# RozDavid/UnScene3D

Hardware: AMD Instinct MI355X
Metric: training scenes/sec (Res16UNet34C+Mask3D, 150k voxels) (higher is better)
Workload: dtype f32

## Files before the change

include/usc3d.h:

```cpp
#ifndef USC3D_H
#define USC3D_H

#include <stdint.h>

#ifdef __cplusplus
extern "C" {
#endif

typedef void* usc_stream_t;

enum usc_status {
  USC_OK = 0,
  USC_ERR_ARG = -1,
  USC_ERR_LAUNCH = -2,
  USC_ERR_RANGE = -3
};

const char* usc_last_error(void);
int usc_abi_version(void);
const char* usc_build_info(void);
int usc_device_count(void);


int usc_voxel_floor_f64(const double* xyz, int64_t n, double voxel_size,
// ... 288 lines not shown
                         void* ws, int64_t ws_bytes, usc_stream_t s);
int usc_bn_backward_reduce(const float* x, const float* dy, const float* y_out,
                           const float* mean, const float* invstd, int64_t n,
                           int32_t c, int32_t training, int32_t accumulate, float* dgamma,
                           float* dbeta, float* mean_g, float* mean_gxhat,
                           void* ws, int64_t ws_bytes, usc_stream_t s);
int usc_relu_fwd(const float* x, float* y, int64_t numel, usc_stream_t s);
int usc_relu_bwd(const float* y, const float* dy, float* dx, int64_t numel,
                 usc_stream_t s);

int usc_avgpool_down2(const float* in, int32_t c, const int32_t* nbr2,
                      int64_t n_coarse, float* out, usc_stream_t s);
int usc_avgpool_down2_ex(const float* in, int32_t c, int32_t ld,
                         const int64_t* row_of, const int32_t* nbr2,
                         int64_t n_coarse, float* out, uint8_t* mask_out,
                         usc_stream_t s);

int usc_gather_rows(const float* src, int32_t c, const int64_t* idx, int64_t n,
                    float* out, usc_stream_t s);

int usc_scatter_add_rows(const float* src, int32_t c, const int64_t* idx,
                         int64_t n, float* dst, usc_stream_t s);

int usc_scatter_rows_unique(const float* src, int32_t c, const int64_t* idx,
                            int64_t n, float* dst, usc_stream_t s);
int usc_scatter_rows_unique_add(const float* src, int32_t c, const int64_t* idx,
                                int64_t n, float* dst, usc_stream_t s);

int64_t usc_sample_keys_ws_bytes(int32_t n_scenes, int32_t K, int32_t q);
int usc_sample_keys(const float* feats, int32_t c, const uint8_t* mask, int32_t q, const float* pos, int32_t p,
                    const int64_t* idx, int32_t n_scenes, int32_t K, const int32_t* n_valid, float* out_feats,
                    uint8_t* out_mask, float* out_pos, void* ws, int64_t ws_bytes, usc_stream_t s);

int64_t usc_segment_csr_ws_bytes(int64_t n, int64_t S);
int usc_segment_csr(const int64_t* seg, int64_t n, int64_t S, int64_t* order,
                    int64_t* seg_off, void* ws, int64_t ws_bytes,
                    usc_stream_t s);
int usc_segment_mean_fwd(const float* src, int32_t c, const int64_t* order,
                         const int64_t* seg_off, int64_t S, float* out,
                         usc_stream_t s);
int usc_segment_mean_bwd(const float* dout, int32_t c, const int64_t* seg,
                         const int64_t* seg_off, int64_t n, float* dsrc,
                         usc_stream_t s);

int usc_segment_mean_nonzero(const float* feats, int32_t d,
                             const int64_t* order, const int64_t* seg_off,
                             int64_t S, float* out, int64_t* nonzero_cnt,
                             usc_stream_t s);
int usc_segment_max_nonzero(const float* feats, int32_t d,
                            const int64_t* order, const int64_t* seg_off,
                            int64_t S, float* out, int64_t* nonzero_cnt,
                            usc_stream_t s);

int32_t usc_attn_max_queries(void);
int32_t usc_attn_lse_stride(int32_t L);
int64_t usc_attn_ws_bytes(int32_t L, int32_t S, int32_t B, int32_t H);
int usc_attn_fwd(const float* q, const float* k, const float* v,
                 const uint8_t* mask, int32_t L, int32_t S, int32_t B, int32_t H,
                 int32_t E, float* o, float* lse, void* ws, int64_t ws_bytes,
                 usc_stream_t s);
int usc_attn_bwd(const float* q, const float* k, const float* v,
                 const uint8_t* mask, const float* o, const float* lse,
                 const float* dO, int32_t L, int32_t S, int32_t B, int32_t H,
                 int32_t E, float* dq, float* dk, float* dv,
                 int32_t mask_bits_in_ws ,
                 void* ws, int64_t ws_bytes, usc_stream_t s);
// ... 329 lines not shown
```

unscene3d_amd/_lib.py:

```python
from __future__ import annotations

import ctypes as C
import os

import torch

_HERE = os.path.dirname(os.path.abspath(__file__))
LIB_PATH = os.environ.get("USC3D_LIB") or os.path.join(_HERE, "libusc3d_hip.so")

_p = C.c_void_p
_i32 = C.c_int32
_i64 = C.c_int64
_f64 = C.c_double
_f32 = C.c_float

class KMap(C.Structure):
    _fields_ = [("nbr", _p), ("perm", _p), ("tile_mask", _p), ("pair_in", _p), ("pair_out", _p), ("koff", _p),
                ("n_in", _i64), ("n_out", _i64), ("pair_capacity", _i64), ("K", _i32), ("reserved", _i32)]


class BNDesc(C.Structure):
    _fields_ = [("gamma", _p), ("beta", _p), ("running_mean", _p), ("running_var", _p), ("num_batches_tracked", _p),
                ("eps", _f32), ("momentum", _f32), ("c", _i32), ("training", _i32)]

# ... 81 lines not shown
    "usc_launch_stats_begin": (C.c_int, [_p, _i64, _p]),
    "usc_launch_stats_end": (_i64, [_p, _i64]),
    "usc_wall_clock_khz": (_i64, []),
    "usc_conv_ws_bytes": (_i64, [_kp, _i32, _i32, _i32]),
    "usc_unit_ws_bytes": (_i64, [_kp, _i32, _i32, _i32]),
    "usc_conv_forward": (C.c_int, [_kp, _i32, _p, _i32, _p, _i32, _p, _p, _p, _i64, _p]),
    "usc_conv_backward": (C.c_int, [_kp, _i32, _p, _i32, _p, _i32, _p, _p, _i32, _p, _i32, _p, _i64, _p]),
    "usc_bn_eval_stats": (C.c_int, [_p, _p, _p, _p, _f32, _i32, _p, _p, _p, _p, _p]),
    "usc_conv_bn_act_forward": (C.c_int, [_kp, _i32, _p, _i32, _p, _i32, _bp, _p, _i32, _p, _p, _p, _p, _i64, _p]),
    "usc_unit_bf16_ws_bytes": (_i64, [_kp, _i32, _i32, _i32]),
    "usc_conv_bn_act_forward_bf16": (C.c_int, [_kp, _i32, _p, _i32, _p, _i32, _bp, _p, _i32, _p, _p, _p, _p, _i64, _p]),
    "usc_unit_split_ws_bytes": (_i64, [_kp, _i32, _i32, _i32, _i32]),
    "usc_conv_bn_act_forward_split": (C.c_int, [_kp, _i32, _p, _i32, _p, _i32, _i32, _bp, _p, _i32, _p, _p, _p, _p, _i64, _p]),
    "usc_conv_bn_act_backward_split": (C.c_int, [_kp, _i32, _p, _i32, _p, _i32, _i32, _bp, _p, _p, _p, _p, _p, _p, _p, _i32, _p,
                                                 _i32, _p, _p, _i32, _p, _i64, _p]),
    "usc_conv_bn_act_backward": (C.c_int, [_kp, _i32, _p, _i32, _p, _i32, _bp, _p, _p, _p, _p, _p, _p, _p, _i32, _p,
                                           _i32, _p, _p, _i32, _p, _i64, _p]),
    "usc_colstats_ws_bytes": (_i64, [_i64, _i32]),
    "usc_colstats": (C.c_int, [_p, _p, _i64, _i32, _p, _p, _p, _i64, _p]),
    "usc_bn_apply": (C.c_int, [_p, _p, _p, _p, _i32, _p, _i64, _i32, _p]),
    "usc_bn_backward_dx": (C.c_int, [_p, _p, _p, _p, _p, _p, _p, _p, _p, _p, _i64, _i32, _p]),
    "usc_bn_backward_reduce": (C.c_int, [_p, _p, _p, _p, _p, _i64, _i32, _i32, _i32, _p, _p, _p, _p, _p, _i64, _p]),
    "usc_bn_forward_stats": (C.c_int, [_p, _i64, _i32, _p, _p, _f32, _f32, _p, _p, _p, _p, _p, _p, _p, _p, _i64, _p]),
    "usc_relu_fwd": (C.c_int, [_p, _p, _i64, _p]),
    "usc_relu_bwd": (C.c_int, [_p, _p, _p, _i64, _p]),
    "usc_avgpool_down2": (C.c_int, [_p, _i32, _p, _i64, _p, _p]),
    "usc_avgpool_down2_ex": (C.c_int, [_p, _i32, _i32, _p, _p, _i64, _p, _p, _p]),
    "usc_gather_rows": (C.c_int, [_p, _i32, _p, _i64, _p, _p]),
    "usc_scatter_add_rows": (C.c_int, [_p, _i32, _p, _i64, _p, _p]),
    "usc_scatter_rows_unique": (C.c_int, [_p, _i32, _p, _i64, _p, _p]),
    "usc_scatter_rows_unique_add": (C.c_int, [_p, _i32, _p, _i64, _p, _p]),
    "usc_sample_keys_ws_bytes": (_i64, [_i32, _i32, _i32]),
    "usc_sample_keys": (C.c_int, [_p, _i32, _p, _i32, _p, _i32, _p, _i32, _i32, _p, _p, _p, _p, _p, _i64, _p]),
    "usc_segment_csr_ws_bytes": (_i64, [_i64, _i64]),
    "usc_segment_csr": (C.c_int, [_p, _i64, _i64, _p, _p, _p, _i64, _p]),
    "usc_segment_mean_fwd": (C.c_int, [_p, _i32, _p, _p, _i64, _p, _p]),
    "usc_segment_mean_bwd": (C.c_int, [_p, _i32, _p, _p, _i64, _p, _p]),
    "usc_segment_mean_nonzero": (C.c_int, [_p, _i32, _p, _p, _i64, _p, _p, _p]),
    "usc_segment_max_nonzero": (C.c_int, [_p, _i32, _p, _p, _i64, _p, _p, _p]),
    "usc_ncut_similarity": (C.c_int, [_p, _i64, _i32, _i32, _p, _p, _p]),
    "usc_ncut_similarity_masked": (C.c_int, [_p, _p, _i64, _i32, _i32, _p, _p, _p]),
    "usc_ncut_normalize_mat": (C.c_int, [_p, _i64, _p, _i64, _p]),
    "usc_ncut_binarize": (C.c_int, [_p, _p, _i64, _f32, _f64, _p, _p, _p, _p]),
    "usc_ncut_fiedler_ws_bytes": (_i64, [_i64]),
    "usc_ncut_fiedler": (C.c_int, [_p, _p, _i64, _f64, _p, _p, _p, _i64, _p]),
    "usc_ncut_fiedler_ex": (C.c_int, [_p, _p, _i64, _f64, _p, _p, _p, _i64, _p, _i32]),
    "usc_ncut_fiedler_plan": (_i32, [_i64, _i32, _i32]),
    "usc_knn1": (C.c_int, [_p, _i64, _p, _i64, _p, _p, _p]),
    "usc_knn1_grid_ws_bytes": (_i64, [_i64, _p]),
    "usc_knn1_grid": (C.c_int, [_p, _i64, _p, _i64, _p, _f64, _p, _p, _p, _p, _i64, _p]),
    "usc_knn_hybrid_grid_ws_bytes": (_i64, [_i64, _p]),
    "usc_knn_hybrid_grid": (C.c_int, [_p, _i64, _p, _i64, _f32, _i32, _p, _f64, _p, _p, _p, _p, _i64, _p]),
    "usc_normals_pca": (C.c_int, [_p, _i64, _p, _i64, _p, _p, _i32, _p, _p]),
    "usc_cc_eps_init": (C.c_int, [_p, _i64, _p]),
    "usc_cc_eps_step": (C.c_int, [_p, _i64, _f32, _p, _p, _p, _p]),
    "usc_cc_eps_finish": (C.c_int, [_p, _i64, _p, _p, _p]),
    "usc_dbscan_cell_keys": (C.c_int, [_p, _i64, _f32, _f64, _f64, _f64, _i32, _i32, _i32, _p, _p]),
    "usc_dbscan_neighbor_table": (C.c_int, [_p, _i64, _i32, _i32, _i32, _p, _p]),
    "usc_dbscan_ws_bytes": (_i64, [_i64, _i32, _i64, _i32]),
    "usc_dbscan_labels": (C.c_int, [_p, _p, _p, _p, _p, _p, _i64, _i32, _i64, _f32, _i32, _p, _i64, _p, _p, _p]),
    "usc_dbscan_expand": (C.c_int, [_p, _p, _p, _i64, _i32, _i64, _p, _p]),
    "usc_project_planes_fwd": (C.c_int, [_p, _p, _p, _i64, _i32, _i32, _i32, _i32] + [_p] * 10),
    "usc_project_planes_bwd": (C.c_int, [_p, _i64, _i32, _i32, _i32, _i32, _p, _p, _p, _p, _p]),
    "usc_brick_mask_build": (C.c_int, [_p, _i64, _p, _i32, _i32, _i32, _i32, _p, _p]),
    "usc_raycast_first_hit_map": (C.c_int, [_p, _p, _i64, _i64, _p, _p, _i32, _i32, _i32, _p, _p, _i32, _i32, _i32, _i32,
                                            _f32, _f32, _f32, _p, _p, _p]),
# ... 133 lines not shown
```

unscene3d_amd/csrc/rows.hip:

```cpp
#include <math.h>
#include <stdlib.h>

#include "common.h"
#include "scan.h"

namespace usc {

void launch_group_reduce(const float* partial, int G, int64_t numel4, int cout, const float* bias, int accumulate,
                         float* out, hipStream_t st);

enum StatMode { STAT_XY = 0, STAT_BN_BWD = 1 };

struct StatArgs {
  const float* x;
  const float* y;
  const float* y_out;
  const float* mean;
  const float* invstd;
  int64_t n;
  int c;
};

constexpr int kStatMaxBlocks = 1024;
constexpr int kStatUnroll = 4;
// ... 519 lines not shown
  const int CT = c / VEC;
  const int64_t total = n_coarse * CT;
  for (int64_t j = (int64_t)blockIdx.x * blockDim.x + threadIdx.x; j < total; j += (int64_t)gridDim.x * blockDim.x) {
    const int64_t p = j / CT;
    const int cg = (int)(j - p * CT);
    float acc[VEC];
#pragma unroll
    for (int v = 0; v < VEC; ++v) acc[v] = 0.f;
    int cnt = 0;
#pragma unroll
    for (int k = 0; k < 8; ++k) {
      const int ch = nbr2[(int64_t)k * n_coarse + p];
      if (ch >= 0) {
        ++cnt;
        const int64_t row = row_of ? row_of[ch] : (int64_t)ch;
        if (VEC == 4) {
          const float4 t = *reinterpret_cast<const float4*>(in + row * ld + cg * 4);
          acc[0] += t.x; acc[1] += t.y; acc[2] += t.z; acc[3] += t.w;
        } else {
          acc[0] += in[row * ld + cg];
        }
      }
    }
    const float inv = 1.f / (float)(cnt > 0 ? cnt : 1);
    if (mask_out) {
#pragma unroll
      for (int v = 0; v < VEC; ++v) mask_out[p * c + cg * VEC + v] = (1.f / (1.f + expf(-(acc[v] * inv)))) < 0.5f;
    } else if (VEC == 4) {
      *reinterpret_cast<float4*>(out + p * c + cg * 4) =
          make_float4(acc[0] * inv, acc[1] * inv, acc[2] * inv, acc[3] * inv);
    } else {
      out[p * c + cg] = acc[0] * inv;
    }
  }
}

template <int VEC>
__global__ __launch_bounds__(256) void gather_rows_kernel(const float* __restrict__ src, int c,
                                                         const int64_t* __restrict__ idx, int64_t n,
                                                         float* __restrict__ out) {
  const int CT = c / VEC;
  const int64_t total = n * CT;
  for (int64_t j = (int64_t)blockIdx.x * blockDim.x + threadIdx.x; j < total; j += (int64_t)gridDim.x * blockDim.x) {
    const int64_t r = j / CT;
    const int cg = (int)(j - r * CT);
    const int64_t sr = idx[r];
    if (VEC == 4)
      *reinterpret_cast<float4*>(out + r * c + cg * 4) = *reinterpret_cast<const float4*>(src + sr * c + cg * 4);
    else
      out[r * c + cg] = src[sr * c + cg];
  }
}

constexpr int kSegTile = 1024;

__global__ __launch_bounds__(256) void seg_hist_kernel(const int64_t* __restrict__ seg, int64_t n, int64_t S,
                                                      int32_t* __restrict__ hist ) {
  const int64_t t = blockIdx.x;
  const int64_t b = t * kSegTile;
  for (int j = threadIdx.x; j < kSegTile; j += 256) {
    const int64_t i = b + j;
    if (i < n) atomicAdd(&hist[t * S + seg[i]], 1);
  }
}
__global__ __launch_bounds__(256) void seg_tilescan_kernel(int32_t* __restrict__ hist, int64_t T, int64_t S,
                                                          int32_t* __restrict__ counts) {
// ... 733 lines not shown
  USC_REQUIRE(n_scenes >= 1 && n_scenes <= usc::kSampleMaxScenes && K >= 1 && c >= 0 && c % 4 == 0 && q >= 0 &&
                  c <= 512 && q <= usc::kSampleMaxQ && (pos == nullptr || (p >= 4 && p % 4 == 0 && p <= 512)) &&
                  (c > 0 || q > 0),
              "usc_sample_keys: unsupported sizes (scenes <= 16, queries <= 256, channel counts multiples of 4 up to 512)");
  USC_REQUIRE(idx && n_valid && (c == 0 || (feats && out_feats)) && (q == 0 || (mask && out_mask && ws)) &&
                  (pos == nullptr || out_pos),
              "usc_sample_keys: null pointer");
  if (c == 0) { feats = nullptr; out_feats = nullptr; }
  if (q == 0) { mask = nullptr; out_mask = nullptr; }
  usc::SampleArgs a{};
  a.feats = feats; a.mask = mask; a.pos = pos; a.idx = idx;
  a.out_feats = out_feats; a.out_mask = out_mask; a.out_pos = out_pos; a.part = (unsigned char*)ws;
  a.c = c; a.q = q; a.p = p; a.K = K;
  a.nblk = (int)ceil_div((int64_t)K, (int64_t)usc::kSampleRows);
  a.qs = (q + 3) / 4 * 4;
  USC_REQUIRE(q == 0 || ((uintptr_t)ws & 3) == 0, "usc_sample_keys: workspace must be 4-byte aligned");
  USC_REQUIRE(q == 0 || ws_bytes >= usc_sample_keys_ws_bytes(n_scenes, K, q), "usc_sample_keys: workspace too small");
  for (int b = 0; b < n_scenes; ++b) {
    USC_REQUIRE(n_valid[b] >= 1, "usc_sample_keys: a scene without rows");
    a.n_valid[b] = n_valid[b];
  }
  const dim3 grid((unsigned)a.nblk, (unsigned)n_scenes);
  if (q <= 128) {
    hipLaunchKernelGGL(usc::sample_keys_kernel<1>, grid, dim3(256), 0, as_stream(s), a);
    if (q > 0) hipLaunchKernelGGL(usc::sample_fix_kernel<1>, grid, dim3(256), 0, as_stream(s), a);
  } else {
    hipLaunchKernelGGL(usc::sample_keys_kernel<2>, grid, dim3(256), 0, as_stream(s), a);
    hipLaunchKernelGGL(usc::sample_fix_kernel<2>, grid, dim3(256), 0, as_stream(s), a);
  }
  USC_CHECK_LAUNCH("usc_sample_keys");
  return USC_OK;
}

int usc_scatter_rows_unique(const float* src, int32_t c, const int64_t* idx, int64_t n, float* dst, usc_stream_t s) {
  USC_REQUIRE(c >= 1 && n >= 0, "usc_scatter_rows_unique: bad sizes");
  if (n == 0) return USC_OK;
  USC_REQUIRE(src && idx && dst, "usc_scatter_rows_unique: null pointer");
  if (c % 4 == 0)
    hipLaunchKernelGGL((usc::scatter_rows_kernel<4>), dim3(stream_grid(n * (c / 4), 256)), dim3(256), 0, as_stream(s), src,
                       (int)c, idx, n, dst);
  else
    hipLaunchKernelGGL((usc::scatter_rows_kernel<1>), dim3(stream_grid(n * c, 256)), dim3(256), 0, as_stream(s), src, (int)c,
                       idx, n, dst);
  USC_CHECK_LAUNCH("usc_scatter_rows_unique");
  return USC_OK;
}

int usc_scatter_rows_unique_add(const float* src, int32_t c, const int64_t* idx, int64_t n, float* dst, usc_stream_t s) {
  USC_REQUIRE(c >= 1 && n >= 0, "usc_scatter_rows_unique_add: bad sizes");
  if (n == 0) return USC_OK;
  USC_REQUIRE(src && idx && dst, "usc_scatter_rows_unique_add: null pointer");
  if (c % 4 == 0)
    hipLaunchKernelGGL((usc::scatter_rows_rmw_kernel<4>), dim3(stream_grid(n * (c / 4), 256)), dim3(256), 0, as_stream(s),
                       src, (int)c, idx, n, dst);
  else
    hipLaunchKernelGGL((usc::scatter_rows_rmw_kernel<1>), dim3(stream_grid(n * c, 256)), dim3(256), 0, as_stream(s), src,
                       (int)c, idx, n, dst);
  USC_CHECK_LAUNCH("usc_scatter_rows_unique_add");
  return USC_OK;
}

int usc_scatter_add_rows(const float* src, int32_t c, const int64_t* idx, int64_t n, float* dst, usc_stream_t s) {
  USC_REQUIRE(c >= 1 && n >= 0, "usc_scatter_add_rows: bad sizes");
  if (n == 0) return USC_OK;
  USC_REQUIRE(src && idx && dst, "usc_scatter_add_rows: null pointer");
  if (c % 4 == 0)
// ... 132 lines not shown
```

unscene3d_amd/models/mask3d.py:

```python
import contextlib
import os

import torch
import torch.nn as nn
from torch.nn import functional as F

from .. import MinkowskiEngine as ME
from .. import ops
from ..MinkowskiEngine import MinkowskiOps as me
from ..MinkowskiEngine.MinkowskiPooling import MinkowskiAvgPooling
from ..pointnet2_utils import furthest_point_sample
from .modules.common import conv
from .modules.helpers_3detr import GenericMLP
from .position_embedding import PositionEmbeddingCoordsSine

SINGLE_POINT_ERROR = "only a single point gives nans in cross-attention"


class Mask3D(nn.Module):
    def __init__(self, config, hidden_dim, num_queries, num_heads, dim_feedforward, sample_sizes, shared_decoder,
                 num_classes, num_decoders, dropout, pre_norm, positional_encoding_type, non_parametric_queries,
                 train_on_segments, normalize_pos_enc, use_level_embed, scatter_type, hlevels, use_np_features,
                 voxel_size, max_sample_size, random_queries, gauss_scale, random_query_both, random_normal):
        super().__init__()
# ... 319 lines not shown
                    elif plan["gidx"] is not None:
                        bufs = step_fn.input_buffers
                feats_l = aux[hlevel].F
                fused = (plan["gidx"] is not None and feats_l.is_cuda
                         and feats_l.dtype == torch.float32 and n_scenes <= 16 and feats_l.shape[1] % 4 == 0
                         and self.num_queries <= fused_attn_max_queries())

                on_side = use_side and fused
                if on_side:
                    for t in (plan["gidx"], samples["pos_keys"][pidx], feats_l):
                        if t is not None and t.is_cuda:
                            t.record_stream(side)
                with (torch.cuda.stream(side) if on_side else contextlib.nullcontext()):
                    if fused:
                        batched_aux = ops.sample_keys(
                            feats_l.contiguous(), None, None, plan["gidx"], n_scenes, curr_sample_size, n_valid,
                            unique=plan["all_sampled"], valid_unique=True,
                            sink=sinks.setdefault((hlevel, bool(plan["all_sampled"])), ops.GradSink()))
                    else:
                        batched_aux = _stack([ops.gather_rows(decomposed_aux[k].contiguous(), rand_idx[k],
                                                              unique=sizes[k] > curr_sample_size) for k in range(n_scenes)])
                    k_keys, v_keys = self._key_prep(dec, i)(batched_aux, samples["pos_keys"][pidx],
                                                            outs=None if bufs is None else (bufs[2], bufs[3]))
                    if on_side:
                        kv_done = torch.cuda.Event()
                        kv_done.record(side)
                        if bufs is None:
                            k_keys.record_stream(main)
                            v_keys.record_stream(main)

                normed, queries = self._norm_queries(queries)
                output_class, outputs_mask, attn_mask = self.mask_module(
                    queries, mask_features, mask_segments, len(aux) - hlevel - 1, ret_attn_mask=True,
                    point2segment=p2s_arg, coords=coords, defer_class=True, normed=normed)
                decomposed_attn = attn_mask.decomposed_features
                if fused and attn_mask.F.dtype == torch.bool and attn_mask.F.shape[1] <= fused_attn_max_queries():
                    batched_attn = ops.sample_keys(None, attn_mask.F.contiguous(), None, plan["gidx"], n_scenes,
                                                   curr_sample_size, n_valid,
                                                   outs=None if bufs is None else (None, bufs[4], None))
                else:
                    batched_attn = _stack([decomposed_attn[k][rand_idx[k], :] for k in range(n_scenes)])
                    batched_attn.permute(0, 2, 1)[batched_attn.sum(1) == curr_sample_size] = False
                    if not plan["all_sampled"]:
                        batched_attn = torch.logical_or(batched_attn, _stack(mask_idx)[..., None])
                    if bufs is not None:
                        bufs[4].copy_(batched_attn)
                        batched_attn = bufs[4]

                rec = getattr(self, "attn_mask_record", None)
                if rec is not None:
                    rec.append(batched_attn.detach().clone())
                if on_side:
                    main.wait_event(kv_done)
                queries = step_fn(queries, query_pos, k_keys, v_keys, batched_attn.contiguous())

                predictions_class.append(output_class)
                predictions_mask.append(outputs_mask)

        output_class, outputs_mask = self.mask_module(queries, mask_features, mask_segments, 0, ret_attn_mask=False,
                                                      point2segment=p2s_arg, coords=coords, defer_class=True)
        predictions_class.append(output_class)
        predictions_mask.append(outputs_mask)
        if early is not None:
            predictions_mask = _early_stage_gate(self, early, pcd_features, mask_features, seg_csr, predictions_mask)
        predictions_class = list(self.class_embed_head(torch.stack(predictions_class)).unbind(0))

        return {
            "pred_logits": predictions_class[-1],
            "pred_masks": predictions_mask[-1],
            "aux_outputs": self._set_aux_loss(predictions_class, predictions_mask),
            "sampled_coords": _host_array(sampled_coords) if sampled_coords is not None else None,
            "backbone_features": pcd_features,
        }

    def _early_stage(self, pcd_features, aux, point2segment):
        from .. import program
        feats = pcd_features.F
        handle = program.handle_of(feats)
        if not (self.training and torch.is_grad_enabled() and self.train_on_segments and self.scatter_type == "mean"
                and not self.use_np_features and point2segment is not None and feats.is_cuda
                and feats.dtype == torch.float32 and self.mask_dim % 32 == 0 and (len(aux) - 1) not in self.hlevels
                and program.early_possible(handle)):
            return None
        head = self.mask_features_head
        bias = head.bias
        if head.kernel_volume != 1 or head.stride != 1 or ops._grad_target(head.kernel) is None:
            return None
        if bias is not None and not (bias.requires_grad and ops._grad_target(bias) is not None):
            return None
        cm = pcd_features.coordinate_manager
        if not all(isinstance(sl, slice) for sl in cm.batch_slices(pcd_features._ts())):
            return None
        return handle

    def _norm_queries(self, queries):
        norm = self.decoder_norm
        if (queries.is_cuda and queries.dtype == torch.float32 and queries.requires_grad
                and isinstance(norm, LayerNorm) and norm.elementwise_affine and norm.bias is not None
                and len(norm.normalized_shape) == 1 and norm.normalized_shape[0] in ops._LN_DIMS):
            return ops.layer_norm(queries, norm.weight, norm.bias, norm.eps, passthrough=True)
        return norm(queries), queries

    def mask_module(self, query_feat, mask_features, mask_segments, num_pooling_steps, ret_attn_mask=True,
                    point2segment=None, coords=None, defer_class=False, normed=None):
        query_feat = self.decoder_norm(query_feat) if normed is None else normed
        head = self.mask_embed_head
        Q = query_feat.shape[-2]
        q_pad = (-Q) % 32
        if query_feat.is_cuda and query_feat.dtype == torch.float32:
            if defer_class and query_feat.requires_grad:
                hidden, query_feat = ops.linear(query_feat, head[0].weight, head[0].bias, relu=True, passthrough=True)
            else:
                hidden = ops.linear(query_feat, head[0].weight, head[0].bias, relu=True)
            if (q_pad and query_feat.dim() == 3 and query_feat.shape[0] == 1
                    and isinstance(head[2], Linear) and head[2].out_features % 32 == 0):
                mask_embed = ops.linear(hidden, head[2].weight, head[2].bias, pad_rows_to=Q + q_pad)
                mask_embed = _PaddedRows(mask_embed, Q)
            else:
                mask_embed = head[2](hidden)
        else:
            mask_embed = head(query_feat)
        outputs_class = query_feat if defer_class else self.class_embed_head(query_feat)

        output_masks, output_segments = [], []
        if (point2segment is not None and ret_attn_mask and num_pooling_steps >= 1 and query_feat.is_cuda
                and _FUSED_ATTN_MASK):
            for i, seg_feat in enumerate(mask_segments):
                logits, mask_segments[i] = _mask_logits(seg_feat, mask_embed[i], chain=True)
                output_segments.append(logits)
            cm, ts = mask_features.coordinate_manager, mask_features._ts()
            if len(output_segments) == 1:
                pooled = output_segments[0].detach()
                rows = point2segment[0].to(torch.int64).contiguous()
            else:
                Q = output_segments[0].shape[1]
                pooled = torch.cat([getattr(o, "_usc_padded", o).detach() for o in output_segments])[:, :Q]
                rows = getattr(cm, "_usc_p2s_batched", None)
                if rows is None or rows.shape[0] != mask_features.F.shape[0]:
                    off, parts = 0, []
                    for p2s, seg in zip(point2segment, mask_segments):
                        parts.append(p2s.to(torch.int64) + off)
                        off += seg.shape[0]
                    rows = torch.cat(parts).contiguous()
                    cm._usc_p2s_batched = rows
            for step in range(num_pooling_steps):
                if step == 0:
                    pooled = ops.avgpool_down2(pooled, _child_segment_table(cm, ts, rows),
                                               threshold=num_pooling_steps == 1)
                else:
                    pooled = ops.avgpool_down2(pooled, cm.stride_map(ts)["nbr2"],
                                               threshold=step == num_pooling_steps - 1)
                ts *= 2
            attn_mask = me.SparseTensor(features=pooled, coordinate_manager=cm,
                                        coordinate_map_key=ME.CoordinateMapKey(ts))
            return outputs_class, output_segments, attn_mask
        if point2segment is not None:
            for i, seg_feat in enumerate(mask_segments):
                output_segments.append(_mask_logits(seg_feat, mask_embed[i]))
                if ret_attn_mask:
                    with torch.no_grad():
                        output_masks.append(ops.gather_rows(output_segments[-1].detach().contiguous(),
                                                            point2segment[i].to(torch.int64).contiguous()))
        else:
            per_scene = mask_features.decomposed_features
            for i in range(len(per_scene)):
                output_masks.append(_mask_logits(per_scene[i], mask_embed[i]))

        if ret_attn_mask:
            attn_mask = me.SparseTensor(features=torch.cat(output_masks).detach(),
                                        coordinate_manager=mask_features.coordinate_manager,
                                        coordinate_map_key=mask_features.coordinate_map_key)
            for _ in range(num_pooling_steps):
                attn_mask = self.pooling(attn_mask.float())
            attn_mask = me.SparseTensor(features=(attn_mask.F.detach().sigmoid() < 0.5),
                                        coordinate_manager=attn_mask.coordinate_manager,
                                        coordinate_map_key=attn_mask.coordinate_map_key)
            if point2segment is not None:
                return outputs_class, output_segments, attn_mask
            return outputs_class, output_masks, attn_mask
        if point2segment is not None:
            return outputs_class, output_segments
        return outputs_class, output_masks

    @torch.jit.unused
# ... 232 lines not shown
_KV_SIDE_STREAM = os.environ.get("USC3D_KV_SIDE_STREAM", "1") != "0"


def set_kv_side_stream(on: bool):
    global _KV_SIDE_STREAM
    if torch.cuda.is_available():
        torch.cuda.synchronize()
    _KV_SIDE_STREAM = bool(on)
_FUSED_ATTN_MASK = os.environ.get("USC3D_FUSED_ATTN_MASK", "1") != "0"
_FUSED_ATTN_WIDE = os.environ.get("USC3D_FUSED_ATTN_WIDE", "1") != "0"


def fused_attn_max_queries() -> int:
    return ops.ATTN_MAX_QUERIES if _FUSED_ATTN_WIDE else min(128, ops.ATTN_MAX_QUERIES)


_PAD_CACHE = {}


def _padded_index(n, size, device):
    key = (int(n), int(size), str(device))
    hit = _PAD_CACHE.get(key)
    if hit is None:
        if len(_PAD_CACHE) > 256:
            _PAD_CACHE.clear()
        idx = torch.zeros(size, dtype=torch.long, device=device)
        midx = torch.ones(size, dtype=torch.bool, device=device)
        idx[:n] = torch.arange(n, device=device)
        midx[:n] = False
        hit = _PAD_CACHE[key] = (idx, midx)
    return hit


def _child_segment_table(cm, ts, rows):
    cache = cm.__dict__.setdefault("_usc_child_segments", {})
    hit = cache.get(ts)
    if hit is None or hit[0] != rows.data_ptr():
        nbr2 = cm.stride_map(ts)["nbr2"]
        tab = torch.where(nbr2 >= 0, rows.to(torch.int32)[nbr2.clamp(min=0).long()], nbr2).contiguous()
        hit = cache[ts] = (rows.data_ptr(), tab, rows)
    return hit[1]


def _segment_max(feats, seg, S):
    out = torch.zeros((int(S), feats.shape[1]), dtype=feats.dtype, device=feats.device)
    return out.scatter_reduce(0, seg.to(torch.int64)[:, None].expand(-1, feats.shape[1]), feats, "amax", include_self=False)


def _stack(tensors):
    tensors = list(tensors)
    return tensors[0].unsqueeze(0) if len(tensors) == 1 else torch.stack(tensors)


def _col_minmax(x):
    mn, mx = torch.aminmax(x.t().contiguous(), dim=1)
    return mn, mx


def _residual_norm(layer, tgt, upd):
    norm = layer.norm
    if (not layer.normalize_before and (layer.dropout.p == 0.0 or not layer.training) and tgt.is_cuda and tgt.dtype == torch.float32
            and isinstance(norm, LayerNorm) and norm.elementwise_affine and norm.bias is not None
            and len(norm.normalized_shape) == 1 and norm.normalized_shape[0] in ops._LN_DIMS
            and tgt.shape == upd.shape):
        return ops.add_layer_norm(tgt, upd, norm.weight, norm.bias, norm.eps)
    out = tgt + layer.dropout(upd)
# ... 144 lines not shown
```

unscene3d_amd/ops.py:

```python
from __future__ import annotations

from dataclasses import dataclass

import ctypes
import os
import weakref

import torch

from . import profiler as _prof
from ._lib import check, lib, require_device


def _stream():
    return torch._C._cuda_getCurrentRawStream(torch._C._cuda_getDevice())


def _chk(t: torch.Tensor, dtype, name: str):
    if not isinstance(t, torch.Tensor):
        raise RuntimeError(f"{name} must be a torch.Tensor")
    if not t.is_cuda:
        raise RuntimeError(f"{name} must be a HIP (cuda) tensor — unscene3d_amd has no CPU path")
    if t.dtype != dtype:
        raise RuntimeError(f"{name} must be {dtype}, got {t.dtype}")
# ... 814 lines not shown
        if sink is not None:
            first = sink.buf is None
            if first:
                sink.buf = torch.zeros((ctx.n_src, c), dtype=torch.float32, device=dfeats.device)
                at_end_of_backward(sink, sink._check, outside="skip")
            scatter(sink.buf, add=not first)
            sink.pending -= 1
            if sink.pending > 0:
                return (None,) * 11
            dsrc, sink.buf = sink.buf, None
            return (dsrc,) + (None,) * 10
        dsrc = torch.zeros((ctx.n_src, c), dtype=torch.float32, device=dfeats.device)
        scatter(dsrc, add=False)
        return (dsrc,) + (None,) * 10


def sample_keys(feats, mask, pos, idx, n_scenes, K, n_valid, outs=None, unique=False, sink=None, valid_unique=False):
    if feats is None and mask is None:
        raise RuntimeError("sample_keys: nothing to gather")
    rows = None
    for t, dt, name in ((feats, torch.float32, "feats"), (mask, torch.bool, "mask"), (pos, torch.float32, "pos")):
        if t is not None:
            _chk(t, dt, name)
            if rows is not None and t.shape[0] != rows:
                raise RuntimeError("sample_keys: feats, mask and pos must have the same rows")
            rows = t.shape[0]
    _chk(idx, torch.int64, "idx")
    if idx.shape[0] != n_scenes * K or len(n_valid) != n_scenes:
        raise RuntimeError("sample_keys: inconsistent sizes")
    if mask is not None and mask.shape[1] > ATTN_MAX_QUERIES:
        raise RuntimeError(f"sample_keys: the mask rows take <= {ATTN_MAX_QUERIES} queries")
    return _SampleKeys.apply(feats, mask, pos, idx, int(n_scenes), int(K), list(n_valid), outs, unique, sink,
                             valid_unique)


def gather_rows_i32(src: torch.Tensor, idx: torch.Tensor) -> torch.Tensor:
    _chk(src, torch.int32, "src")
    return _GatherRows.apply(src.view(torch.float32), idx.contiguous(), None, False).view(torch.int32)


@dataclass
class SegmentCSR:
    seg: torch.Tensor
    order: torch.Tensor
    seg_off: torch.Tensor
    S: int


def segment_csr(seg: torch.Tensor, S: int) -> SegmentCSR:
    _chk(seg, torch.int64, "seg")
    n = seg.shape[0]
    dev = seg.device
    order = torch.empty(n, dtype=torch.int64, device=dev)
    seg_off = torch.empty(S + 1, dtype=torch.int64, device=dev)
    ws = _ws(lib.usc_segment_csr_ws_bytes(n, S), dev)
    check(lib.usc_segment_csr(_ptr(seg), n, S, _ptr(order), _ptr(seg_off), _ptr(ws), ws.numel(), _stream()),
          "usc_segment_csr")
    return SegmentCSR(seg, order, seg_off, S)


def segment_sum_from_csr(src, csr: SegmentCSR):
    mean = torch.empty((csr.S, src.shape[1]), dtype=torch.float32, device=src.device)
    check(lib.usc_segment_mean_fwd(_ptr(src), src.shape[1], _ptr(csr.order), _ptr(csr.seg_off), csr.S, _ptr(mean),
                                   _stream()), "usc_segment_mean_fwd")
    cnt = (csr.seg_off[1:] - csr.seg_off[:-1]).to(torch.float32)
    return mean * cnt[:, None]
# ... 996 lines not shown
```

Measured before the change: 46.49.

## Compute attention mask only for sampled key rows via fused hierarchical pooling kernel

Instead of average-pooling the full mask logits through every level and then gathering the sampled keys, a new kernel walks the child tables from each sampled key down to the leaf logits. It averages them level by level in LDS, applies the sigmoid threshold and writes the bool attention mask rows directly, followed by the existing fix-up pass for fully masked columns. This skips pooling rows that are never sampled and removes the intermediate pooled tensors and the separate gather. In exchange, sibling subtrees shared by keys are recomputed, and the fine-level gathers are irregular.

```diff
diff --git a/include/usc3d.h b/include/usc3d.h
--- a/include/usc3d.h
+++ b/include/usc3d.h
@@ -344,6 +344,12 @@
                     const int64_t* idx, int32_t n_scenes, int32_t K, const int32_t* n_valid, float* out_feats,
                     uint8_t* out_mask, float* out_pos, void* ws, int64_t ws_bytes, usc_stream_t s);
 
+int64_t usc_attn_mask_rows_ws_bytes(int32_t n_scenes, int32_t K, int32_t q, int32_t d);
+int usc_attn_mask_rows(const float* in, int32_t ld, int32_t q, int32_t d, const int32_t* const* tabs,
+                       const int64_t* n_rows, const int64_t* idx, int32_t n_scenes, int32_t K,
+                       const int32_t* n_valid, uint8_t* out_mask, void* ws, int64_t ws_bytes, int32_t skip_fix,
+                       usc_stream_t s);
+
 int64_t usc_segment_csr_ws_bytes(int64_t n, int64_t S);
 int usc_segment_csr(const int64_t* seg, int64_t n, int64_t S, int64_t* order,
                     int64_t* seg_off, void* ws, int64_t ws_bytes,
diff --git a/unscene3d_amd/_lib.py b/unscene3d_amd/_lib.py
--- a/unscene3d_amd/_lib.py
+++ b/unscene3d_amd/_lib.py
@@ -137,6 +137,8 @@
     "usc_scatter_rows_unique_add": (C.c_int, [_p, _i32, _p, _i64, _p, _p]),
     "usc_sample_keys_ws_bytes": (_i64, [_i32, _i32, _i32]),
     "usc_sample_keys": (C.c_int, [_p, _i32, _p, _i32, _p, _i32, _p, _i32, _i32, _p, _p, _p, _p, _p, _i64, _p]),
+    "usc_attn_mask_rows_ws_bytes": (_i64, [_i32, _i32, _i32, _i32]),
+    "usc_attn_mask_rows": (C.c_int, [_p, _i32, _i32, _i32, _p, _p, _p, _i32, _i32, _p, _p, _p, _i64, _i32, _p]),
     "usc_segment_csr_ws_bytes": (_i64, [_i64, _i64]),
     "usc_segment_csr": (C.c_int, [_p, _i64, _i64, _p, _p, _p, _i64, _p]),
     "usc_segment_mean_fwd": (C.c_int, [_p, _i32, _p, _p, _i64, _p, _p]),
diff --git a/unscene3d_amd/csrc/rows.hip b/unscene3d_amd/csrc/rows.hip
--- a/unscene3d_amd/csrc/rows.hip
+++ b/unscene3d_amd/csrc/rows.hip
@@ -575,6 +575,185 @@
     } else {
       out[p * c + cg] = acc[0] * inv;
     }
+  }
+}
+
+constexpr int kMaskRowsMaxDepth = 4;
+struct MaskRowsArgs {
+  const float* in; const int64_t* idx; unsigned char* out_mask; unsigned char* part;
+  const int32_t* tab[kMaskRowsMaxDepth];
+  int64_t n[kMaskRowsMaxDepth];
+  int ld, q4, K, nblk;
+  int n_valid[kSampleMaxScenes];
+};
+static constexpr int mask_rows_keys(int d) { return d == 1 ? 64 : d == 2 ? 16 : d == 3 ? 4 : 1; }
+static constexpr int mask_rows_threads(int d) { return d <= 2 ? 512 : 1024; }
+
+__device__ __forceinline__ float4 mask_leaf_mean(const MaskRowsArgs& a, const int (&ids)[8], int c4) {
+#pragma clang fp contract(off)
+  float4 t[8];
+#pragma unroll
+  for (int k = 0; k < 8; ++k)
+    t[k] = *reinterpret_cast<const float4*>(a.in + (int64_t)(ids[k] >= 0 ? ids[k] : 0) * a.ld + c4 * 4);
+  float4 acc = make_float4(0.f, 0.f, 0.f, 0.f);
+  int cnt = 0;
+#pragma unroll
+  for (int k = 0; k < 8; ++k)
+    if (ids[k] >= 0) {
+      ++cnt;
+      acc.x += t[k].x; acc.y += t[k].y; acc.z += t[k].z; acc.w += t[k].w;
+    }
+  const float inv = 1.f / (float)(cnt > 0 ? cnt : 1);
+  float4 m;
+  m.x = acc.x * inv; m.y = acc.y * inv; m.z = acc.z * inv; m.w = acc.w * inv;
+  return m;
+}
+
+template <int L>
+__device__ __forceinline__ float4 mask_node_mean(const MaskRowsArgs& a, int64_t p, int c4) {
+#pragma clang fp contract(off)
+  static_assert(L == 1 || L == 2, "one group walks at most two levels");
+  int ch[8];
+#pragma unroll
+  for (int k = 0; k < 8; ++k) ch[k] = a.tab[L - 1][k * a.n[L - 1] + p];
+  if constexpr (L == 1) {
+    return mask_leaf_mean(a, ch, c4);
+  } else {
+    int leaf[8][8];
+#pragma unroll
+    for (int k = 0; k < 8; ++k)
+#pragma unroll
+      for (int j = 0; j < 8; ++j) leaf[k][j] = a.tab[0][j * a.n[0] + (ch[k] >= 0 ? ch[k] : 0)];
+    float4 acc = make_float4(0.f, 0.f, 0.f, 0.f);
+    int cnt = 0;
+#pragma unroll
+    for (int k = 0; k < 8; ++k) {
+      const float4 m = mask_leaf_mean(a, leaf[k], c4);
+      if (ch[k] >= 0) {
+        ++cnt;
+        acc.x += m.x; acc.y += m.y; acc.z += m.z; acc.w += m.w;
+      }
+    }
+    const float inv = 1.f / (float)(cnt > 0 ? cnt : 1);
+    float4 m;
+    m.x = acc.x * inv; m.y = acc.y * inv; m.z = acc.z * inv; m.w = acc.w * inv;
+    return m;
+  }
+}
+
+__device__ __forceinline__ unsigned int mask_rows_bit(float mean) {
+  return (1.f / (1.f + expf(-mean))) < 0.5f ? 1u : 0u;
+}
+
+template <int D>
+__global__ __launch_bounds__(mask_rows_threads(D)) void attn_mask_rows_kernel(MaskRowsArgs a) {
+#pragma clang fp contract(off)
+  constexpr int NT = mask_rows_threads(D), NG = NT / 32;
+  constexpr int S = D <= 2 ? 0 : D - 2, L = D - S, R = mask_rows_keys(D);
+  constexpr int NI = S == 0 ? 1 : (S == 1 ? R * 8 : 64);
+  static_assert(S < 2 || R == 1, "two LDS levels: one key per workgroup");
+  static_assert(NI <= NT && NG >= 8, "one thread per item; one group per child of the key");
+  __shared__ int leaf[D == 1 ? R : 1][8];
+  __shared__ float4 val[NI][32];
+  __shared__ float4 val2[S == 2 ? 8 : 1][32];
+  __shared__ int node[NI];
+  __shared__ int node2[8];
+  __shared__ unsigned int band[R][32];
+  const int t = threadIdx.x, c4 = t & 31, g = t >> 5;
+  const int b = blockIdx.y, k0 = blockIdx.x * R;
+  const bool col = c4 < a.q4;
+  const int64_t* __restrict__ idx = a.idx + (int64_t)b * a.K;
+
+  if constexpr (D == 1) {
+    for (int e = t; e < R * 8; e += NT) {
+      const int r = e >> 3, k = e & 7;
+      leaf[r][k] = k0 + r < a.K ? a.tab[0][k * a.n[0] + idx[k0 + r]] : -1;
+    }
+    __syncthreads();
+  }
+  if constexpr (S >= 1) {
+    if (t < NI) {
+      const int r = S == 1 ? t >> 3 : 0, k = S == 1 ? t & 7 : t >> 3;
+      int nd = -1;
+      if (k0 + r < a.K) {
+        nd = a.tab[D - 1][k * a.n[D - 1] + idx[k0 + r]];
+        if constexpr (S == 2) {
+          if ((t & 7) == 0) node2[k] = nd;
+          if (nd >= 0) nd = a.tab[D - 2][(t & 7) * a.n[D - 2] + nd];
+        }
+      }
+      node[t] = nd;
+    }
+    __syncthreads();
+    for (int it = g; it < NI; it += NG) {
+      const int nd = node[it];
+      if (nd >= 0 && col) val[it][c4] = mask_node_mean<L>(a, nd, c4);
+    }
+    __syncthreads();
+    if constexpr (S == 2) {
+      if (g < 8 && node2[g] >= 0 && col) {
+        float4 acc = make_float4(0.f, 0.f, 0.f, 0.f);
+        int cnt = 0;
+#pragma unroll
+        for (int k = 0; k < 8; ++k)
+          if (node[g * 8 + k] >= 0) {
+            ++cnt;
+            const float4 v = val[g * 8 + k][c4];
+            acc.x += v.x; acc.y += v.y; acc.z += v.z; acc.w += v.w;
+          }
+        const float inv = 1.f / (float)(cnt > 0 ? cnt : 1);
+        float4 m;
+        m.x = acc.x * inv; m.y = acc.y * inv; m.z = acc.z * inv; m.w = acc.w * inv;
+        val2[g][c4] = m;
+      }
+      __syncthreads();
+    }
+  }
+
+#pragma unroll 4
+  for (int r = g; r < R; r += NG) {
+    const int kk = k0 + r;
+    unsigned int word = 0x01010101u;
+    if (kk < a.K && col) {
+      float4 m;
+      if constexpr (D == 1) {
+        m = mask_leaf_mean(a, leaf[r], c4);
+      } else if constexpr (S == 0) {
+        m = mask_node_mean<L>(a, idx[kk], c4);
+      } else {
+        float4 acc = make_float4(0.f, 0.f, 0.f, 0.f);
+        int cnt = 0;
+#pragma unroll
+        for (int k = 0; k < 8; ++k) {
+          bool present;
+          float4 v;
+          if constexpr (S == 1) {
+            present = node[r * 8 + k] >= 0;
+            v = val[r * 8 + k][c4];
+          } else {
+            present = node2[k] >= 0;
+            v = val2[k][c4];
+          }
+          if (present) {
+            ++cnt;
+            acc.x += v.x; acc.y += v.y; acc.z += v.z; acc.w += v.w;
+          }
+        }
+        const float inv = 1.f / (float)(cnt > 0 ? cnt : 1);
+        m.x = acc.x * inv; m.y = acc.y * inv; m.z = acc.z * inv; m.w = acc.w * inv;
+      }
+      word = mask_rows_bit(m.x) | (mask_rows_bit(m.y) << 8) | (mask_rows_bit(m.z) << 16) | (mask_rows_bit(m.w) << 24);
+      reinterpret_cast<unsigned int*>(a.out_mask + ((int64_t)b * a.K + kk) * (a.q4 * 4))[c4] =
+          kk >= a.n_valid[b] ? 0x01010101u : word;
+    }
+    band[r][c4] = word;
+  }
+  __syncthreads();
+  if (t < a.q4) {
+    unsigned int w = band[0][t];
+#pragma unroll
+    for (int r = 1; r < R; ++r) w &= band[r][t];
+    reinterpret_cast<unsigned int*>(a.part + ((int64_t)b * a.nblk + blockIdx.x) * (a.q4 * 4))[t] = w;
   }
 }
 
@@ -1374,6 +1553,59 @@
   return USC_OK;
 }
 
+int64_t usc_attn_mask_rows_ws_bytes(int32_t n_scenes, int32_t K, int32_t q, int32_t d) {
+  if (d < 1 || d > usc::kMaskRowsMaxDepth || n_scenes < 1 || K < 1 || q < 0) return -1;
+  return (int64_t)n_scenes * ceil_div((int64_t)K, (int64_t)usc::mask_rows_keys(d)) * ((q + 3) / 4 * 4);
+}
+
+int usc_attn_mask_rows(const float* in, int32_t ld, int32_t q, int32_t d, const int32_t* const* tabs,
+                       const int64_t* n_rows, const int64_t* idx, int32_t n_scenes, int32_t K,
+                       const int32_t* n_valid, uint8_t* out_mask, void* ws, int64_t ws_bytes, int32_t skip_fix,
+                       usc_stream_t s) {
+  USC_REQUIRE(d >= 1 && d <= usc::kMaskRowsMaxDepth, "usc_attn_mask_rows: %d pooling steps (1..%d)", d,
+              usc::kMaskRowsMaxDepth);
+  USC_REQUIRE(q >= 4 && q % 4 == 0 && q <= 128, "usc_attn_mask_rows: %d queries (a multiple of 4, <= 128)", q);
+  USC_REQUIRE(n_scenes >= 1 && n_scenes <= usc::kSampleMaxScenes && K >= 1,
+              "usc_attn_mask_rows: unsupported sizes (1..16 scenes, K >= 1)");
+  USC_REQUIRE(ld >= q && ld % 4 == 0, "usc_attn_mask_rows: leading dimension %d (a multiple of 4, >= q)", ld);
+  USC_REQUIRE(in && tabs && n_rows && idx && n_valid && out_mask && ws, "usc_attn_mask_rows: null pointer");
+  USC_REQUIRE(((uintptr_t)in & 15) == 0 && ((uintptr_t)out_mask & 3) == 0 && ((uintptr_t)ws & 3) == 0,
+              "usc_attn_mask_rows: logits must be 16-byte aligned, mask rows and workspace 4-byte aligned");
+  usc::MaskRowsArgs a{};
+  for (int j = 0; j < d; ++j) {
+    USC_REQUIRE(tabs[j] != nullptr, "usc_attn_mask_rows: child table %d is null", j);
+    USC_REQUIRE(n_rows[j] >= 1 && n_rows[j] <= INT32_MAX, "usc_attn_mask_rows: child table %d has %lld rows", j,
+                (long long)n_rows[j]);
+    a.tab[j] = tabs[j];
+    a.n[j] = n_rows[j];
+  }
+  USC_REQUIRE(ws_bytes >= usc_attn_mask_rows_ws_bytes(n_scenes, K, q, d), "usc_attn_mask_rows: workspace too small");
+  for (int b = 0; b < n_scenes; ++b) {
+    USC_REQUIRE(n_valid[b] >= 1, "usc_attn_mask_rows: a scene without rows");
+    a.n_valid[b] = n_valid[b];
+  }
+  a.in = in; a.idx = idx; a.out_mask = out_mask; a.part = (unsigned char*)ws;
+  a.ld = ld; a.q4 = q / 4; a.K = K;
+  a.nblk = (int)ceil_div((int64_t)K, (int64_t)usc::mask_rows_keys(d));
+  const dim3 grid((unsigned)a.nblk, (unsigned)n_scenes);
+  switch (d) {
+    case 1: hipLaunchKernelGGL(usc::attn_mask_rows_kernel<1>, grid, dim3(usc::mask_rows_threads(1)), 0, as_stream(s), a); break;
+    case 2: hipLaunchKernelGGL(usc::attn_mask_rows_kernel<2>, grid, dim3(usc::mask_rows_threads(2)), 0, as_stream(s), a); break;
+    case 3: hipLaunchKernelGGL(usc::attn_mask_rows_kernel<3>, grid, dim3(usc::mask_rows_threads(3)), 0, as_stream(s), a); break;
+    default: hipLaunchKernelGGL(usc::attn_mask_rows_kernel<4>, grid, dim3(usc::mask_rows_threads(4)), 0, as_stream(s), a); break;
+  }
+  if (!skip_fix) {
+    usc::SampleArgs f{};
+    f.out_mask = out_mask; f.part = (unsigned char*)ws;
+    f.q = q; f.qs = q; f.K = K; f.nblk = a.nblk;
+    for (int b = 0; b < n_scenes; ++b) f.n_valid[b] = n_valid[b];
+    const dim3 fgrid((unsigned)ceil_div((int64_t)K, (int64_t)usc::kSampleRows), (unsigned)n_scenes);
+    hipLaunchKernelGGL(usc::sample_fix_kernel<1>, fgrid, dim3(256), 0, as_stream(s), f);
+  }
+  USC_CHECK_LAUNCH("usc_attn_mask_rows");
+  return USC_OK;
+}
+
 int usc_scatter_rows_unique(const float* src, int32_t c, const int64_t* idx, int64_t n, float* dst, usc_stream_t s) {
   USC_REQUIRE(c >= 1 && n >= 0, "usc_scatter_rows_unique: bad sizes");
   if (n == 0) return USC_OK;
diff --git a/unscene3d_amd/models/mask3d.py b/unscene3d_amd/models/mask3d.py
--- a/unscene3d_amd/models/mask3d.py
+++ b/unscene3d_amd/models/mask3d.py
@@ -375,13 +375,16 @@
                 normed, queries = self._norm_queries(queries)
                 output_class, outputs_mask, attn_mask = self.mask_module(
                     queries, mask_features, mask_segments, len(aux) - hlevel - 1, ret_attn_mask=True,
-                    point2segment=p2s_arg, coords=coords, defer_class=True, normed=normed)
-                decomposed_attn = attn_mask.decomposed_features
-                if fused and attn_mask.F.dtype == torch.bool and attn_mask.F.shape[1] <= fused_attn_max_queries():
+                    point2segment=p2s_arg, coords=coords, defer_class=True, normed=normed, sampled_rows_only=fused)
+                if isinstance(attn_mask, _AttnMaskRows):
+                    batched_attn = ops.attn_mask_rows(attn_mask.logits, attn_mask.tables, plan["gidx"], n_scenes,
+                                                      curr_sample_size, n_valid, outs=None if bufs is None else bufs[4])
+                elif fused and attn_mask.F.dtype == torch.bool and attn_mask.F.shape[1] <= fused_attn_max_queries():
                     batched_attn = ops.sample_keys(None, attn_mask.F.contiguous(), None, plan["gidx"], n_scenes,
                                                    curr_sample_size, n_valid,
                                                    outs=None if bufs is None else (None, bufs[4], None))
                 else:
+                    decomposed_attn = attn_mask.decomposed_features
                     batched_attn = _stack([decomposed_attn[k][rand_idx[k], :] for k in range(n_scenes)])
                     batched_attn.permute(0, 2, 1)[batched_attn.sum(1) == curr_sample_size] = False
                     if not plan["all_sampled"]:
@@ -445,7 +448,7 @@
         return norm(queries), queries
 
     def mask_module(self, query_feat, mask_features, mask_segments, num_pooling_steps, ret_attn_mask=True,
-                    point2segment=None, coords=None, defer_class=False, normed=None):
+                    point2segment=None, coords=None, defer_class=False, normed=None, sampled_rows_only=False):
         query_feat = self.decoder_norm(query_feat) if normed is None else normed
         head = self.mask_embed_head
         Q = query_feat.shape[-2]
@@ -486,13 +489,12 @@
                         off += seg.shape[0]
                     rows = torch.cat(parts).contiguous()
                     cm._usc_p2s_batched = rows
-            for step in range(num_pooling_steps):
-                if step == 0:
-                    pooled = ops.avgpool_down2(pooled, _child_segment_table(cm, ts, rows),
-                                               threshold=num_pooling_steps == 1)
-                else:
-                    pooled = ops.avgpool_down2(pooled, cm.stride_map(ts)["nbr2"],
-                                               threshold=step == num_pooling_steps - 1)
+            tables = [_child_segment_table(cm, ts, rows)]
+            tables += [cm.stride_map(ts << step)["nbr2"] for step in range(1, num_pooling_steps)]
+            if sampled_rows_only and ops.attn_mask_rows_applies(pooled, tables, len(mask_segments)):
+                return outputs_class, output_segments, _AttnMaskRows(pooled, tables)
+            for step, table in enumerate(tables):
+                pooled = ops.avgpool_down2(pooled, table, threshold=step == num_pooling_steps - 1)
                 ts *= 2
             attn_mask = me.SparseTensor(features=pooled, coordinate_manager=cm,
                                         coordinate_map_key=ME.CoordinateMapKey(ts))
@@ -791,6 +793,13 @@
     return hit
 
 
+class _AttnMaskRows:
+    __slots__ = ("logits", "tables")
+
+    def __init__(self, logits, tables):
+        self.logits, self.tables = logits, tables
+
+
 def _child_segment_table(cm, ts, rows):
     cache = cm.__dict__.setdefault("_usc_child_segments", {})
     hit = cache.get(ts)
diff --git a/unscene3d_amd/ops.py b/unscene3d_amd/ops.py
--- a/unscene3d_amd/ops.py
+++ b/unscene3d_amd/ops.py
@@ -870,6 +870,47 @@
         raise RuntimeError(f"sample_keys: the mask rows take <= {ATTN_MAX_QUERIES} queries")
     return _SampleKeys.apply(feats, mask, pos, idx, int(n_scenes), int(K), list(n_valid), outs, unique, sink,
                              valid_unique)
+
+
+ATTN_MASK_ROWS_MAX_QUERIES = 128
+ATTN_MASK_ROWS_MAX_STEPS = 4
+
+
+def attn_mask_rows_applies(logits, tables, n_scenes) -> bool:
+    q = logits.shape[1]
+    ld = logits.stride(0) if logits.shape[0] > 1 else q
+    return (logits.is_cuda and logits.dtype == torch.float32 and logits.dim() == 2 and logits.stride(1) == 1
+            and q % 4 == 0 and 4 <= q <= ATTN_MASK_ROWS_MAX_QUERIES and ld % 4 == 0 and logits.data_ptr() % 16 == 0
+            and 1 <= len(tables) <= ATTN_MASK_ROWS_MAX_STEPS and 1 <= n_scenes <= 16)
+
+
+def attn_mask_rows(logits, tables, idx, n_scenes, K, n_valid, outs=None, fix=True):
+    if not attn_mask_rows_applies(logits, tables, n_scenes):
+        raise RuntimeError("attn_mask_rows: f32 HIP logits with 4..128 queries (a multiple of 4), a leading dimension "
+                           "that is a multiple of 4, 1..4 child tables and <= 16 scenes")
+    _chk(idx, torch.int64, "idx")
+    q, d, dev = logits.shape[1], len(tables), logits.device
+    for t in tables:
+        _chk(t, torch.int32, "child table")
+        if t.dim() != 2 or t.shape[0] != 8 or t.shape[1] < 1:
+            raise RuntimeError("attn_mask_rows: a child table must be i32 [8, n]")
+    if idx.shape[0] != n_scenes * K or len(n_valid) != n_scenes:
+        raise RuntimeError("attn_mask_rows: inconsistent sizes")
+    if outs is None:
+        out = torch.empty((n_scenes, K, q), dtype=torch.bool, device=dev)
+    else:
+        out = outs.detach()
+        if tuple(out.shape) != (n_scenes, K, q) or out.dtype != torch.bool or not out.is_contiguous():
+            raise RuntimeError(f"attn_mask_rows: the mask buffer {tuple(out.shape)} {out.dtype} does not fit "
+                               f"{(n_scenes, K, q)} contiguous bool")
+    ld = logits.stride(0) if logits.shape[0] > 1 else q
+    tabs = (ctypes.c_void_p * d)(*[t.data_ptr() for t in tables])
+    rows = (ctypes.c_int64 * d)(*[t.shape[1] for t in tables])
+    nv = (ctypes.c_int32 * n_scenes)(*[int(v) for v in n_valid])
+    ws = _ws(lib.usc_attn_mask_rows_ws_bytes(n_scenes, K, q, d), dev)
+    check(lib.usc_attn_mask_rows(_ptr(logits), ld, q, d, tabs, rows, _ptr(idx), n_scenes, K, nv, _ptr(out), _ptr(ws),
+                                 ws.numel(), 0 if fix else 1, _stream()), "usc_attn_mask_rows")
+    return out
 
 
 def gather_rows_i32(src: torch.Tensor, idx: torch.Tensor) -> torch.Tensor:
```

Result: faster. 47.23 (median of 6 runs) (+1.6%).
